# Boese0601/RC-MVSNet

Hardware: AMD Instinct MI355X
Metric: ref-scenes/sec (DTU 3-view 512x640, D=48/32/8) (higher is better)
Workload: dtype f32; 1 GPU; BASELINE configs[1]: CascadeMVSNet_eval.forward, DTU-shaped 3 views 512x640, D=(48,32,8), batch 1 per GPU, fp32, random-init seeded weights; views=3, height=512, width=640, parallelism=scene-per-gpu x1, ranks=1, procs_per_gpu=1, rccl_ranks=0

## Files before the change

### rc_mvsnet_amd/csrc/conv3d_deep.hip

```cpp
#include "common.h"
#include "x3_pieces.h"
#include <atomic>
#include <type_traits>

namespace rcmvs {

enum { DP_S1 = 0, DP_S2 = 1, DP_T2 = 2 };

__host__ __device__ constexpr int dp_ntaps(int p) { return (((p >> 2) & 1) + 1) * (((p >> 1) & 1) + 1) * ((p & 1) + 1); }
__host__ __device__ constexpr int dp_first_sum(int p) { int s = 0; for (int q = 0; q < p; ++q) s += dp_ntaps(q); return s; }
__host__ __device__ constexpr int dp_first(int p) { return (int)((0x130F0B0905030100ull >> (8 * p)) & 0xffu); }
static_assert(dp_first(1) == dp_first_sum(1) && dp_first(2) == dp_first_sum(2) && dp_first(3) == dp_first_sum(3) && dp_first(4) == dp_first_sum(4) &&
              dp_first(5) == dp_first_sum(5) && dp_first(6) == dp_first_sum(6) && dp_first(7) == dp_first_sum(7) && dp_first(0) == 0, "class offsets");
__host__ __device__ inline void dp_class_tap(int p, int i, int& kd, int& kh, int& kw) {
    const int pd = (p >> 2) & 1, ph = (p >> 1) & 1, pw = p & 1;
    const int iw = i & pw, ih = (i >> pw) & ph, id = (i >> (pw + ph)) & pd;
    kd = pd ? 2 * id : 1; kh = ph ? 2 * ih : 1; kw = pw ? 2 * iw : 1;
}

template <int CIN, int COUT, int KIND, int MS = 1>
struct Deep {
    static constexpr int NT = 2;
    static constexpr int TH = 2 * NT, TW = 8;
    static constexpr int MT = COUT / 16;
    static constexpr int HALVES = CIN >= 32 ? CIN / 32 : 1;
    static constexpr int TPS = CIN >= 32 ? 1 : 32 / CIN;
    static constexpr int HD = KIND == DP_T2 ? 2 : 3;
    static constexpr int HH = KIND == DP_S1 ? TH + 2 : (KIND == DP_S2 ? 2 * TH + 1 : TH + 1);
    static constexpr int HW = KIND == DP_S1 ? TW + 2 : (KIND == DP_S2 ? 2 * TW + 1 : TW + 1);
    static constexpr int CS = KIND == DP_S2 ? 2 : 1;
    static constexpr int NVOX = HD * HH * HW;
    static constexpr int VS = CIN * 2 + 16;
    static constexpr int PLANE = NVOX * VS;
    static constexpr int KSTEPS = (27 + TPS - 1) / TPS * HALVES;
    static constexpr int UNITS = NVOX * (CIN / 8);
    static constexpr int NLD = (UNITS + 511) / 512;
    static constexpr int PF = KIND == DP_T2 ? 6 : 8;
    static constexpr int MSPLIT = (KIND != DP_T2 && MT == 4) ? MS : 1;
    static constexpr int MB = MT / MSPLIT;
    static constexpr int KP = KIND == DP_T2 ? 1 : 8 / MB;
    static constexpr int PARTB = KIND == DP_T2 ? 0 : (KP - 1) * MB * NT * 1024;
    static constexpr int LDS = 2 * PLANE + PARTB + 64;
    static constexpr long long IMG_HALFS = 8 + (long long)KSTEPS * 2 * MT * 512;
    static_assert((CIN % 32 == 0 || (CIN == 16 && KIND != DP_T2)) && COUT % 16 == 0 && (KIND == DP_T2 ? (MT == 2 || MT == 1) : (MT == 4 || MT == 2)), "wave layout");
};

template <int CIN, int COUT, int KIND>
__global__ void deep_pack_kernel(const float* __restrict__ w, unsigned short* __restrict__ img, int transposed, const float* __restrict__ wsc) {
    using C = Deep<CIN, COUT, KIND>;
    const int t = blockIdx.x * blockDim.x + threadIdx.x;
    if (t >= C::KSTEPS * C::MT * 512) return;
    const int e = t & 7, lane = (t >> 3) & 63, mt = (t >> 9) % C::MT, j = (t >> 9) / C::MT;
    const int co = mt * 16 + (lane & 15), kq = lane >> 4;
    int tap, half;
    if (KIND == DP_T2) {
        int p = 0;
        while (p < 7 && j >= dp_first(p + 1) * C::HALVES) ++p;
        const int jj = j - dp_first(p) * C::HALVES;
        int kd, kh, kw;
        dp_class_tap(p, jj / C::HALVES, kd, kh, kw);
        tap = (kd * 3 + kh) * 3 + kw;
        half = jj % C::HALVES;
    } else if (C::TPS == 2) { tap = 2 * j + (kq >> 1); half = 0; }
    else { tap = j / C::HALVES; half = j % C::HALVES; }
    const int ci = C::TPS == 2 ? (kq & 1) * 8 + e : half * 32 + kq * 8 + e;
    float v = 0.0f;
    if (tap < 27) v = transposed ? w[((long long)ci * COUT + co) * 27 + (transposed == 2 ? 26 - tap : tap)] : w[((long long)co * CIN + ci) * 27 + tap];
    const float sw = wsc[0];
    if (t == 0) { float* hdr = reinterpret_cast<float*>(img); hdr[0] = sw; hdr[1] = wsc[1]; hdr[2] = 0.0f; hdr[3] = 0.0f; }
    const float vs = v * sw;
    const _Float16 h = (_Float16)vs;
    const _Float16 l = (_Float16)(vs - (float)h);
    const long long base = 8 + (((long long)j * 2) * C::MT + mt) * 512 + lane * 8 + e;
    img[base] = __builtin_bit_cast(unsigned short, h);
    img[base + (long long)C::MT * 512] = __builtin_bit_cast(unsigned short, l);
}

struct DeepDims {
    int B, D, H, W;
    int Dg, Hg, Wg;
    int Do, Ho, Wo;
    int tiles_h, tiles_w, relu;
};

__device__ __forceinline__ int dp_t2_segments(int wave, int (&cls)[3]) {
    const int g = wave >> 1;
    cls[0] = g == 0 ? 7 : (g == 1 ? 3 : (g == 2 ? 5 : 6));
    cls[1] = g == 1 ? 1 : (g == 2 ? 2 : 4);
    cls[2] = 0;
    return g == 0 ? 1 : (g == 1 ? 3 : 2);
}

template <int CIN, int COUT, int KIND, int MS = 1>
__global__ __launch_bounds__(512) void conv3d_deep_kernel(
    const float* __restrict__ x, const x3_u32x4* __restrict__ wimg, const float* __restrict__ scale, const float* __restrict__ shift,
    const float* __restrict__ res, float* __restrict__ y, DeepDims dm, const float* __restrict__ xmax, float* __restrict__ ymax) {
    using C = Deep<CIN, COUT, KIND, MS>;
    constexpr int MT = C::MT, NT = C::NT, PF = C::PF, VS = C::VS, PLANE = C::PLANE, HALVES = C::HALVES;
    constexpr int OOB = 0x7ffffff0;
    extern __shared__ __attribute__((aligned(16))) x3_byte smem[];
    x3_byte* const part = smem + 2 * PLANE;
    float* const redmax = reinterpret_cast<float*>(part + C::PARTB);
    const int tid = threadIdx.x, lane = tid & 63;
    const int wave = __builtin_amdgcn_readfirstlane(tid >> 6);
    const int n = lane & 15, kq = lane >> 4;
    int bt = blockIdx.x;
    const int tw = bt % dm.tiles_w; bt /= dm.tiles_w;
    const int th = bt % dm.tiles_h; bt /= dm.tiles_h;
    const int dg = bt % dm.Dg, b = bt / dm.Dg;
    const int h0 = th * C::TH, w0 = tw * C::TW;
    const int zd0 = KIND == DP_S1 ? dg - 1 : (KIND == DP_S2 ? 2 * dg - 1 : dg);
    const int zh0 = KIND == DP_S1 ? h0 - 1 : (KIND == DP_S2 ? 2 * h0 - 1 : h0);
    const int zw0 = KIND == DP_S1 ? w0 - 1 : (KIND == DP_S2 ? 2 * w0 - 1 : w0);
    const float xmax_lane = xmax[lane * 16];
    const float whdr = reinterpret_cast<const float*>(wimg)[1];

    int seg_cls[3] = {0, 0, 0}, nseg = 1, mt0;
    if constexpr (KIND == DP_T2 && MT == 1) { seg_cls[0] = wave; mt0 = 0; }
    else if constexpr (KIND == DP_T2) { nseg = dp_t2_segments(wave, seg_cls); mt0 = wave & 1; }
    else mt0 = blockIdx.y * C::MB + wave % C::MB;
    const int kp = KIND == DP_T2 ? 0 : wave / C::MB;
    const int mtl = KIND == DP_T2 ? 0 : wave % C::MB;
    auto seg_range = [&](int sg, int& j0, int& nsteps) {
        if constexpr (KIND == DP_T2) {
            const int cls = seg_cls[sg], nt = dp_ntaps(cls);
            const bool drop = (cls & 4) && zd0 + 1 >= dm.D;
            j0 = (dp_first(cls) + (drop ? nt / 2 : 0)) * HALVES;
            nsteps = (drop ? nt / 2 : nt) * HALVES;
        } else {
            const int lo = (zd0 < 0 ? 9 : 0) * HALVES / C::TPS, hi = ((zd0 + 2 >= dm.D ? 18 : 27) * HALVES + C::TPS - 1) / C::TPS, per = (hi - lo + C::KP - 1) / C::KP;
            j0 = min(lo + kp * per, hi);
            nsteps = min(per, hi - j0);
        }
    };
    auto tap_offset = [&](int cls, int j) -> int {
        const int half = j % HALVES;
        int od, oh, ow;
        if constexpr (KIND == DP_T2) {
            int kd, kh, kw;
            dp_class_tap(cls, j / HALVES - dp_first(cls), kd, kh, kw);
            od = kd == 0; oh = kh == 0; ow = kw == 0;
        } else { const int tp = j / HALVES; od = tp / 9; oh = (tp / 3) % 3; ow = tp % 3; }
        return ((od * C::HH + oh) * C::HW + ow) * VS + half * 64;
    };
    auto tap_offset_of = [&](int tp) -> int { tp = min(tp, 26); return (((tp / 9) * C::HH + (tp / 3) % 3) * C::HW + tp % 3) * VS; };

    __amdgpu_buffer_rsrc_t wrs = __builtin_amdgcn_make_buffer_rsrc(const_cast<x3_u32x4*>(wimg + 1), (short)0, (int)(C::KSTEPS * 2 * MT * 1024), 0x00020000);
    constexpr int NR = KIND == DP_T2 ? 2 : 1;
    x3_u32x4 ah[NR][PF], al[NR][PF];
    const int alane = lane * 16 + mt0 * 1024;
    auto load_a = [&](auto ring, int slot, int j0, int nsteps, int jj) {
        constexpr int R = decltype(ring)::value;
        const int so = (j0 + jj) * (2 * MT * 1024);
        const int vo = jj < nsteps ? alane : OOB;
        ah[R][slot] = __builtin_amdgcn_raw_buffer_load_b128(wrs, vo, so, 0);
        al[R][slot] = __builtin_amdgcn_raw_buffer_load_b128(wrs, vo == OOB ? OOB : vo + MT * 1024, so, 0);
    };
    using Ring0 = std::integral_constant<int, 0>;
    using Ring1 = std::integral_constant<int, NR - 1>;

    float unscale;
    {
        __amdgpu_buffer_rsrc_t xrs = __builtin_amdgcn_make_buffer_rsrc(const_cast<float*>(x), (short)0,
                                                                       (int)((long long)dm.B * dm.D * dm.H * dm.W * CIN * 4), 0x00020000);
        x3_f32x4 pf[C::NLD][2];
        int lo_[C::NLD];
#pragma unroll
        for (int i = 0; i < C::NLD; ++i) {
            const int u = tid + i * 512;
            const int vox = u / (CIN / 8), cu = u % (CIN / 8);
            const int hw_ = vox % C::HW, hh = (vox / C::HW) % C::HH, hd = vox / (C::HW * C::HH);
            const int id = zd0 + hd, ih = zh0 + hh, iw = zw0 + hw_;
            const bool in = u < C::UNITS && id >= 0 && id < dm.D && ih >= 0 && ih < dm.H && iw >= 0 && iw < dm.W;
            const int off = in ? ((((b * dm.D + id) * dm.H + ih) * dm.W + iw) * CIN + cu * 8) * 4 : OOB;
            pf[i][0] = __builtin_bit_cast(x3_f32x4, __builtin_amdgcn_raw_buffer_load_b128(xrs, off, 0, 0));
            pf[i][1] = __builtin_bit_cast(x3_f32x4, __builtin_amdgcn_raw_buffer_load_b128(xrs, in ? off + 16 : OOB, 0, 0));
            lo_[i] = u < C::UNITS ? vox * VS + cu * 16 : -1;
        }
        {
            int j0, nsteps;
            seg_range(0, j0, nsteps);
#pragma unroll
            for (int u = 0; u < PF; ++u) load_a(Ring0{}, u, j0, nsteps, u);
        }
        float bound = xmax_lane;
#pragma unroll
        for (int m = 32; m > 0; m >>= 1) bound = fmaxf(bound, __shfl_xor(bound, m));
        float xinv;
        const float xs_scale = x3_pow2_scale(bound, xinv);
        unscale = xinv * whdr;
#pragma unroll
        for (int i = 0; i < C::NLD; ++i) {
            x3_u32x2 h0_, l0_, h1_, l1_;
            x3_split4h(pf[i][0] * xs_scale, h0_, l0_);
            x3_split4h(pf[i][1] * xs_scale, h1_, l1_);
            if (lo_[i] >= 0) {
                *reinterpret_cast<x3_u32x4*>(smem + lo_[i]) = (x3_u32x4){h0_.x, h0_.y, h1_.x, h1_.y};
                *reinterpret_cast<x3_u32x4*>(smem + PLANE + lo_[i]) = (x3_u32x4){l0_.x, l0_.y, l1_.x, l1_.y};
            }
        }
    }
    __syncthreads();

    static_assert(PF % 2 == 0, "the B double buffer alternates with the step parity");
    int bb[NT];
#pragma unroll
    for (int t = 0; t < NT; ++t) bb[t] = (((2 * t + (n >> 3)) * C::CS) * C::HW + (n & 7) * C::CS) * VS + (C::TPS == 2 ? (kq & 1) : kq) * 16;
    float vmax = 0.0f;
#pragma unroll
    for (int sg = 0; sg < (KIND == DP_T2 ? 3 : 1); ++sg) {
        if (sg >= nseg) break;
        const int cls = seg_cls[sg];
        int j0, nsteps;
        seg_range(sg, j0, nsteps);
        x3_f32x4 acc[NT][3];
#pragma unroll
        for (int t = 0; t < NT; ++t)
#pragma unroll
            for (int c = 0; c < 3; ++c) acc[t][c] = (x3_f32x4){0.f, 0.f, 0.f, 0.f};
        x3_u32x4 bq[2][NT][2];
        const int jl = j0 + min(lane, nsteps - 1);
        const int entv = C::TPS == 2 ? tap_offset_of(2 * jl) : tap_offset(cls, jl);
        const int entv2 = C::TPS == 2 ? tap_offset_of(2 * jl + 1) : 0;
        auto read_b = [&](int buf, int jj) {
            int boff = __builtin_amdgcn_readlane(entv, jj);
            if constexpr (C::TPS == 2) { const int b2 = __builtin_amdgcn_readlane(entv2, jj); boff = (kq >> 1) ? b2 : boff; }
#pragma unroll
            for (int t = 0; t < NT; ++t) {
                bq[buf][t][0] = *reinterpret_cast<const x3_u32x4*>(smem + bb[t] + boff);
                bq[buf][t][1] = *reinterpret_cast<const x3_u32x4*>(smem + PLANE + bb[t] + boff);
            }
        };
        auto run = [&](auto ring, auto other) {
            constexpr int R = decltype(ring)::value;
            if (sg + 1 < nseg) {
                int j0n, nn;
                seg_range(sg + 1, j0n, nn);
#pragma unroll
                for (int u = 0; u < PF; ++u) load_a(other, u, j0n, nn, u);
            }
            auto mfmas = [&](int slot, int buf) {
#pragma unroll
                for (int t = 0; t < NT; ++t) {
                    acc[t][0] = x3_mfma<2>(ah[R][slot], bq[buf][t][0], acc[t][0]);
                    acc[t][1] = x3_mfma<2>(ah[R][slot], bq[buf][t][1], acc[t][1]);
                    acc[t][2] = x3_mfma<2>(al[R][slot], bq[buf][t][0], acc[t][2]);
                }
            };
            read_b(0, 0);
            int base = 0;
            for (; base + PF <= nsteps; base += PF) {
#pragma unroll
                for (int u = 0; u < PF; ++u) {
                    read_b((u + 1) & 1, base + u + 1);
                    __builtin_amdgcn_sched_barrier(0);
                    mfmas(u, u & 1);
                    __builtin_amdgcn_sched_barrier(0);
                    load_a(ring, u, j0, nsteps, base + u + PF);
                }
            }
#pragma unroll
            for (int u = 0; u < PF; ++u)
                if (base + u < nsteps) {
                    read_b((u + 1) & 1, base + u + 1);
                    __builtin_amdgcn_sched_barrier(0);
                    mfmas(u, u & 1);
                    __builtin_amdgcn_sched_barrier(0);
                }
        };
        if (NR == 1 || !(sg & 1)) run(Ring0{}, Ring1{});
        else run(Ring1{}, Ring0{});

        x3_f32x4 tot[NT];
#pragma unroll
        for (int t = 0; t < NT; ++t) tot[t] = acc[t][0] + (acc[t][1] + acc[t][2]);
        bool finisher = true;
        if constexpr (KIND != DP_T2) {
            finisher = kp == 0;
            if (!finisher) {
#pragma unroll
                for (int t = 0; t < NT; ++t) *reinterpret_cast<x3_f32x4*>(part + ((((kp - 1) * C::MB + mtl) * NT + t) * 64 + lane) * 16) = tot[t];
            }
            __syncthreads();
            if (finisher) {
#pragma unroll
                for (int q = 0; q < C::KP - 1; ++q)
#pragma unroll
                    for (int t = 0; t < NT; ++t) tot[t] += *reinterpret_cast<const x3_f32x4*>(part + (((q * C::MB + mtl) * NT + t) * 64 + lane) * 16);
            }
        }
        if (finisher) {
            const int pd = (cls >> 2) & 1, ph = (cls >> 1) & 1, pw = cls & 1;
            const int co = mt0 * 16 + kq * 4;
            x3_f32x4 sc = (x3_f32x4){unscale, unscale, unscale, unscale}, sh = (x3_f32x4){0.f, 0.f, 0.f, 0.f};
            if (scale) {
                sc = *reinterpret_cast<const x3_f32x4*>(scale + co) * unscale;
                sh = *reinterpret_cast<const x3_f32x4*>(shift + co);
            }
#pragma unroll
            for (int t = 0; t < NT; ++t) {
                const int ch = h0 + 2 * t + (n >> 3), cw = w0 + (n & 7);
                if (ch >= dm.Hg || cw >= dm.Wg) continue;
                const int od = KIND == DP_T2 ? 2 * dg + pd : dg, oh = KIND == DP_T2 ? 2 * ch + ph : ch, ow = KIND == DP_T2 ? 2 * cw + pw : cw;
                const long long ov = ((((long long)b * dm.Do + od) * dm.Ho + oh) * dm.Wo + ow) * COUT + co;
                x3_f32x4 v = tot[t] * sc + sh;
                if (dm.relu) v = __builtin_elementwise_max(v, (x3_f32x4){0.f, 0.f, 0.f, 0.f});
                if (res) v += *reinterpret_cast<const x3_f32x4*>(res + ov);
                *reinterpret_cast<x3_f32x4*>(y + ov) = v;
                vmax = x3_absmax4(vmax, v);
            }
        }
    }
    if (ymax) {
#pragma unroll
        for (int m = 32; m > 0; m >>= 1) vmax = fmaxf(vmax, __shfl_xor(vmax, m));
        if (lane == 0) redmax[wave] = vmax;
        __syncthreads();
        if (tid == 0) {
            float m = redmax[0];
#pragma unroll
            for (int i = 1; i < 8; ++i) m = fmaxf(m, redmax[i]);
            atomicMax(reinterpret_cast<unsigned int*>(ymax) + (blockIdx.x & 63) * 16, __float_as_uint(m));
        }
    }
}

#define RCMVS_DEEP_LIST(X) X(32, 64, DP_S2) X(64, 64, DP_S1) X(64, 32, DP_T2) X(32, 32, DP_S1) X(32, 16, DP_T2) X(16, 32, DP_S2)

bool conv3d_deep_supported(int Ci, int Co, int kind) {
    if (Ci == 16 && Co == 32) {
        static const bool on = [] { const char* e = getenv("RCMVS_DEEP3"); return !e || e[0] != '0'; }();
        if (!on) return false;
    }
    if (Ci == 32 && Co == 16) {
        static const bool on = [] { const char* e = getenv("RCMVS_DEEP9"); return !e || e[0] != '0'; }();
        if (!on) return false;
    }
    if (Ci == 32 && Co == 32) {
        static const bool on = [] { const char* e = getenv("RCMVS_DEEP4"); return !e || e[0] != '0'; }();
        if (!on) return false;
    }
#define DP_CASE(CI, CO, K) if (Ci == CI && Co == CO && kind == K) return true;
    RCMVS_DEEP_LIST(DP_CASE)
#undef DP_CASE
    return false;
}

long long conv3d_deep_weight_floats(int Ci, int Co, int kind) {
#define DP_CASE(CI, CO, K) if (Ci == CI && Co == CO && kind == K) return Deep<CI, CO, K>::IMG_HALFS / 2;
    RCMVS_DEEP_LIST(DP_CASE)
#undef DP_CASE
    return 0;
}

int conv3d_deep_pack(const float* w, float* img, int Co, int Ci, int kind, int transposed, const float* wsc, hipStream_t st) {
#define DP_CASE(CI, CO, K) if (Ci == CI && Co == CO && kind == K) { \
        const int nthr = Deep<CI, CO, K>::KSTEPS * Deep<CI, CO, K>::MT * 512; \
        hipLaunchKernelGGL((deep_pack_kernel<CI, CO, K>), dim3((nthr + 255) / 256), dim3(256), 0, st, w, reinterpret_cast<unsigned short*>(img), transposed, wsc); \
        return launch_status("conv3d_deep_pack"); }
    RCMVS_DEEP_LIST(DP_CASE)
#undef DP_CASE
    return fail(-1, "conv3d_deep_pack: unsupported Ci=%d Co=%d kind=%d", Ci, Co, kind);
}

template <int CI, int CO, int K, int MS>
static int deep_launch_ms(const float* x, const float* wimg, const float* scale, const float* shift, const float* res, float* y,
                          const DeepDims& dm, long long blocks, int dev, const float* xmax, float* ymax, hipStream_t st) {
    using C = Deep<CI, CO, K, MS>;
    constexpr int MAXDEV = 64;
    static std::atomic<bool> raised[MAXDEV];
    if (C::LDS > 64 * 1024 && !raised[dev].load(std::memory_order_acquire)) {
        if (hipFuncSetAttribute((const void*)conv3d_deep_kernel<CI, CO, K, MS>, hipFuncAttributeMaxDynamicSharedMemorySize, C::LDS) != hipSuccess)
            return fail(-1, "conv3d_deep: cannot raise the dynamic LDS limit to %d bytes", C::LDS);
        raised[dev].store(true, std::memory_order_release);
    }
    hipLaunchKernelGGL((conv3d_deep_kernel<CI, CO, K, MS>), dim3((unsigned)blocks, C::MSPLIT), dim3(512), C::LDS, st, x, reinterpret_cast<const x3_u32x4*>(wimg),
                       scale, shift, res, y, dm, xmax, ymax);
    return launch_status("conv3d_deep");
}

template <int CI, int CO, int K>
static int deep_launch_t(const float* x, const float* wimg, const float* scale, const float* shift, const float* res, float* y,
                         const DeepDims& dm_in, int dev, const float* xmax, float* ymax, hipStream_t st) {
    using C = Deep<CI, CO, K>;
    DeepDims dm = dm_in;
    dm.tiles_h = (dm.Hg + C::TH - 1) / C::TH; dm.tiles_w = (dm.Wg + C::TW - 1) / C::TW;
    const long long blocks = (long long)dm.B * dm.Dg * dm.tiles_h * dm.tiles_w;
    if (blocks <= 0 || blocks > 0x7fffffffLL) return fail(-1, "conv3d_deep: bad grid");
    if constexpr (K != DP_T2 && CO == 64) {
        static std::atomic<int> cu_of[64];
        if (cu_of[dev] == 0) {
            hipDeviceProp_t prop;
            cu_of[dev] = (hipGetDeviceProperties(&prop, dev) == hipSuccess && prop.multiProcessorCount > 0) ? prop.multiProcessorCount : 256;
        }
        if (2 * blocks <= cu_of[dev].load()) return deep_launch_ms<CI, CO, K, 2>(x, wimg, scale, shift, res, y, dm, blocks, dev, xmax, ymax, st);
    }
    return deep_launch_ms<CI, CO, K, 1>(x, wimg, scale, shift, res, y, dm, blocks, dev, xmax, ymax, st);
}

int conv3d_deep_launch(const float* x, const float* wimg, const float* scale, const float* shift, const float* res, float* y,
                       int B, int D, int H, int W, int Ci, int Co, int kind, int relu, hipStream_t st, const float* xmax, float* ymax) {
    if (!xmax) return fail(-1, "conv3d_deep: the fp16-pair form needs a bound of max|x|");
    DeepDims dm;
    dm.B = B; dm.D = D; dm.H = H; dm.W = W; dm.relu = relu;
    if (kind == DP_T2) { dm.Do = 2 * D; dm.Ho = 2 * H; dm.Wo = 2 * W; dm.Dg = D; dm.Hg = H; dm.Wg = W; }
    else {
        const int s = kind == DP_S2 ? 2 : 1;
        dm.Do = (D - 1) / s + 1; dm.Ho = (H - 1) / s + 1; dm.Wo = (W - 1) / s + 1;
        dm.Dg = dm.Do; dm.Hg = dm.Ho; dm.Wg = dm.Wo;
    }
    if ((long long)B * D * H * W * Ci * 4 >= 0x7ffffff0LL) return fail(-1, "conv3d_deep: input tensor too large for 32-bit offsets");
    dm.tiles_h = dm.tiles_w = 0;
    int dev = 0;
    if (hipGetDevice(&dev) != hipSuccess || dev < 0 || dev >= 64) return fail(-1, "conv3d_deep: cannot query the device");
#define DP_CASE(CI, CO, K) if (Ci == CI && Co == CO && kind == K) return deep_launch_t<CI, CO, K>(x, wimg, scale, shift, res, y, dm, dev, xmax, ymax, st);
    RCMVS_DEEP_LIST(DP_CASE)
#undef DP_CASE
    return fail(-1, "conv3d_deep: unsupported Ci=%d Co=%d kind=%d", Ci, Co, kind);
}

}
```

Before: 982.1 ref-scenes/s.

## Re-layout deep conv3d LDS planes with row padding to cut bank conflicts

Moves the Deep tile config into a shared header and changes the LDS activation-plane layout. It adds per-row padding and a per-CIN voxel stride, de-interleaves even and odd columns for the stride-2 CIN=32 case, and remaps the global-load unit order so LDS writes group better. The goal is to reduce LDS bank conflicts in the B-operand reads and the staging writes of the MFMA conv. It also adds a host-side bank-conflict model header, used only for analysis. The cost is extra LDS footprint from padding, which may lower occupancy, plus more complex index arithmetic in the load loop.

```diff
diff --git a/rc_mvsnet_amd/csrc/conv3d_deep.hip b/rc_mvsnet_amd/csrc/conv3d_deep.hip
--- a/rc_mvsnet_amd/csrc/conv3d_deep.hip
+++ b/rc_mvsnet_amd/csrc/conv3d_deep.hip
@@ -1,49 +1,10 @@
 #include "common.h"
 #include "x3_pieces.h"
+#include "deep_lds.h"
 #include <atomic>
 #include <type_traits>
 
 namespace rcmvs {
-
-enum { DP_S1 = 0, DP_S2 = 1, DP_T2 = 2 };
-
-__host__ __device__ constexpr int dp_ntaps(int p) { return (((p >> 2) & 1) + 1) * (((p >> 1) & 1) + 1) * ((p & 1) + 1); }
-__host__ __device__ constexpr int dp_first_sum(int p) { int s = 0; for (int q = 0; q < p; ++q) s += dp_ntaps(q); return s; }
-__host__ __device__ constexpr int dp_first(int p) { return (int)((0x130F0B0905030100ull >> (8 * p)) & 0xffu); }
-static_assert(dp_first(1) == dp_first_sum(1) && dp_first(2) == dp_first_sum(2) && dp_first(3) == dp_first_sum(3) && dp_first(4) == dp_first_sum(4) &&
-              dp_first(5) == dp_first_sum(5) && dp_first(6) == dp_first_sum(6) && dp_first(7) == dp_first_sum(7) && dp_first(0) == 0, "class offsets");
-__host__ __device__ inline void dp_class_tap(int p, int i, int& kd, int& kh, int& kw) {
-    const int pd = (p >> 2) & 1, ph = (p >> 1) & 1, pw = p & 1;
-    const int iw = i & pw, ih = (i >> pw) & ph, id = (i >> (pw + ph)) & pd;
-    kd = pd ? 2 * id : 1; kh = ph ? 2 * ih : 1; kw = pw ? 2 * iw : 1;
-}
-
-template <int CIN, int COUT, int KIND, int MS = 1>
-struct Deep {
-    static constexpr int NT = 2;
-    static constexpr int TH = 2 * NT, TW = 8;
-    static constexpr int MT = COUT / 16;
-    static constexpr int HALVES = CIN >= 32 ? CIN / 32 : 1;
-    static constexpr int TPS = CIN >= 32 ? 1 : 32 / CIN;
-    static constexpr int HD = KIND == DP_T2 ? 2 : 3;
-    static constexpr int HH = KIND == DP_S1 ? TH + 2 : (KIND == DP_S2 ? 2 * TH + 1 : TH + 1);
-    static constexpr int HW = KIND == DP_S1 ? TW + 2 : (KIND == DP_S2 ? 2 * TW + 1 : TW + 1);
-    static constexpr int CS = KIND == DP_S2 ? 2 : 1;
-    static constexpr int NVOX = HD * HH * HW;
-    static constexpr int VS = CIN * 2 + 16;
-    static constexpr int PLANE = NVOX * VS;
-    static constexpr int KSTEPS = (27 + TPS - 1) / TPS * HALVES;
-    static constexpr int UNITS = NVOX * (CIN / 8);
-    static constexpr int NLD = (UNITS + 511) / 512;
-    static constexpr int PF = KIND == DP_T2 ? 6 : 8;
-    static constexpr int MSPLIT = (KIND != DP_T2 && MT == 4) ? MS : 1;
-    static constexpr int MB = MT / MSPLIT;
-    static constexpr int KP = KIND == DP_T2 ? 1 : 8 / MB;
-    static constexpr int PARTB = KIND == DP_T2 ? 0 : (KP - 1) * MB * NT * 1024;
-    static constexpr int LDS = 2 * PLANE + PARTB + 64;
-    static constexpr long long IMG_HALFS = 8 + (long long)KSTEPS * 2 * MT * 512;
-    static_assert((CIN % 32 == 0 || (CIN == 16 && KIND != DP_T2)) && COUT % 16 == 0 && (KIND == DP_T2 ? (MT == 2 || MT == 1) : (MT == 4 || MT == 2)), "wave layout");
-};
 
 template <int CIN, int COUT, int KIND>
 __global__ void deep_pack_kernel(const float* __restrict__ w, unsigned short* __restrict__ img, int transposed, const float* __restrict__ wsc) {
@@ -96,7 +57,7 @@
     const float* __restrict__ x, const x3_u32x4* __restrict__ wimg, const float* __restrict__ scale, const float* __restrict__ shift,
     const float* __restrict__ res, float* __restrict__ y, DeepDims dm, const float* __restrict__ xmax, float* __restrict__ ymax) {
     using C = Deep<CIN, COUT, KIND, MS>;
-    constexpr int MT = C::MT, NT = C::NT, PF = C::PF, VS = C::VS, PLANE = C::PLANE, HALVES = C::HALVES;
+    constexpr int MT = C::MT, NT = C::NT, PF = C::PF, PLANE = C::PLANE, HALVES = C::HALVES;
     constexpr int OOB = 0x7ffffff0;
     extern __shared__ __attribute__((aligned(16))) x3_byte smem[];
     x3_byte* const part = smem + 2 * PLANE;
@@ -141,9 +102,9 @@
             dp_class_tap(cls, j / HALVES - dp_first(cls), kd, kh, kw);
             od = kd == 0; oh = kh == 0; ow = kw == 0;
         } else { const int tp = j / HALVES; od = tp / 9; oh = (tp / 3) % 3; ow = tp % 3; }
-        return ((od * C::HH + oh) * C::HW + ow) * VS + half * 64;
+        return C::tap_off(od, oh, ow, half);
     };
-    auto tap_offset_of = [&](int tp) -> int { tp = min(tp, 26); return (((tp / 9) * C::HH + (tp / 3) % 3) * C::HW + tp % 3) * VS; };
+    auto tap_offset_of = [&](int tp) -> int { tp = min(tp, 26); return C::tap_off(tp / 9, (tp / 3) % 3, tp % 3, 0); };
 
     __amdgpu_buffer_rsrc_t wrs = __builtin_amdgcn_make_buffer_rsrc(const_cast<x3_u32x4*>(wimg + 1), (short)0, (int)(C::KSTEPS * 2 * MT * 1024), 0x00020000);
     constexpr int NR = KIND == DP_T2 ? 2 : 1;
@@ -167,15 +128,15 @@
         int lo_[C::NLD];
 #pragma unroll
         for (int i = 0; i < C::NLD; ++i) {
-            const int u = tid + i * 512;
-            const int vox = u / (CIN / 8), cu = u % (CIN / 8);
-            const int hw_ = vox % C::HW, hh = (vox / C::HW) % C::HH, hd = vox / (C::HW * C::HH);
+            int hr, hw_, cu;
+            const bool live = C::unit(tid + i * 512, hr, hw_, cu);
+            const int hh = hr % C::HH, hd = hr / C::HH;
             const int id = zd0 + hd, ih = zh0 + hh, iw = zw0 + hw_;
-            const bool in = u < C::UNITS && id >= 0 && id < dm.D && ih >= 0 && ih < dm.H && iw >= 0 && iw < dm.W;
+            const bool in = live && id >= 0 && id < dm.D && ih >= 0 && ih < dm.H && iw >= 0 && iw < dm.W;
             const int off = in ? ((((b * dm.D + id) * dm.H + ih) * dm.W + iw) * CIN + cu * 8) * 4 : OOB;
             pf[i][0] = __builtin_bit_cast(x3_f32x4, __builtin_amdgcn_raw_buffer_load_b128(xrs, off, 0, 0));
             pf[i][1] = __builtin_bit_cast(x3_f32x4, __builtin_amdgcn_raw_buffer_load_b128(xrs, in ? off + 16 : OOB, 0, 0));
-            lo_[i] = u < C::UNITS ? vox * VS + cu * 16 : -1;
+            lo_[i] = live ? C::vox_off(hr, hw_, cu) : -1;
         }
         {
             int j0, nsteps;
@@ -205,7 +166,7 @@
     static_assert(PF % 2 == 0, "the B double buffer alternates with the step parity");
     int bb[NT];
 #pragma unroll
-    for (int t = 0; t < NT; ++t) bb[t] = (((2 * t + (n >> 3)) * C::CS) * C::HW + (n & 7) * C::CS) * VS + (C::TPS == 2 ? (kq & 1) : kq) * 16;
+    for (int t = 0; t < NT; ++t) bb[t] = C::cell_off(t, n, C::TPS == 2 ? (kq & 1) : kq);
     float vmax = 0.0f;
 #pragma unroll
     for (int sg = 0; sg < (KIND == DP_T2 ? 3 : 1); ++sg) {
@@ -279,14 +240,14 @@
             finisher = kp == 0;
             if (!finisher) {
 #pragma unroll
-                for (int t = 0; t < NT; ++t) *reinterpret_cast<x3_f32x4*>(part + ((((kp - 1) * C::MB + mtl) * NT + t) * 64 + lane) * 16) = tot[t];
+                for (int t = 0; t < NT; ++t) *reinterpret_cast<x3_f32x4*>(part + C::part_off(kp - 1, mtl, t, lane)) = tot[t];
             }
             __syncthreads();
             if (finisher) {
 #pragma unroll
                 for (int q = 0; q < C::KP - 1; ++q)
 #pragma unroll
-                    for (int t = 0; t < NT; ++t) tot[t] += *reinterpret_cast<const x3_f32x4*>(part + (((q * C::MB + mtl) * NT + t) * 64 + lane) * 16);
+                    for (int t = 0; t < NT; ++t) tot[t] += *reinterpret_cast<const x3_f32x4*>(part + C::part_off(q, mtl, t, lane));
             }
         }
         if (finisher) {
diff --git a/rc_mvsnet_amd/csrc/deep_lds.h b/rc_mvsnet_amd/csrc/deep_lds.h
--- /dev/null
+++ b/rc_mvsnet_amd/csrc/deep_lds.h
@@ -0,0 +1,78 @@
+#pragma once
+
+#ifndef __HIPCC__
+#ifndef __host__
+#define __host__
+#endif
+#ifndef __device__
+#define __device__
+#endif
+#endif
+
+namespace rcmvs {
+
+enum { DP_S1 = 0, DP_S2 = 1, DP_T2 = 2 };
+
+__host__ __device__ constexpr int dp_ntaps(int p) { return (((p >> 2) & 1) + 1) * (((p >> 1) & 1) + 1) * ((p & 1) + 1); }
+__host__ __device__ constexpr int dp_first_sum(int p) { int s = 0; for (int q = 0; q < p; ++q) s += dp_ntaps(q); return s; }
+__host__ __device__ constexpr int dp_first(int p) { return (int)((0x130F0B0905030100ull >> (8 * p)) & 0xffu); }
+static_assert(dp_first(1) == dp_first_sum(1) && dp_first(2) == dp_first_sum(2) && dp_first(3) == dp_first_sum(3) && dp_first(4) == dp_first_sum(4) &&
+              dp_first(5) == dp_first_sum(5) && dp_first(6) == dp_first_sum(6) && dp_first(7) == dp_first_sum(7) && dp_first(0) == 0, "class offsets");
+__host__ __device__ inline void dp_class_tap(int p, int i, int& kd, int& kh, int& kw) {
+    const int pd = (p >> 2) & 1, ph = (p >> 1) & 1, pw = p & 1;
+    const int iw = i & pw, ih = (i >> pw) & ph, id = (i >> (pw + ph)) & pd;
+    kd = pd ? 2 * id : 1; kh = ph ? 2 * ih : 1; kw = pw ? 2 * iw : 1;
+}
+
+template <int CIN, int COUT, int KIND, int MS = 1>
+struct Deep {
+    static constexpr int NT = 2;
+    static constexpr int TH = 2 * NT, TW = 8;
+    static constexpr int MT = COUT / 16;
+    static constexpr int HALVES = CIN >= 32 ? CIN / 32 : 1;
+    static constexpr int TPS = CIN >= 32 ? 1 : 32 / CIN;
+    static constexpr int HD = KIND == DP_T2 ? 2 : 3;
+    static constexpr int HH = KIND == DP_S1 ? TH + 2 : (KIND == DP_S2 ? 2 * TH + 1 : TH + 1);
+    static constexpr int HW = KIND == DP_S1 ? TW + 2 : (KIND == DP_S2 ? 2 * TW + 1 : TW + 1);
+    static constexpr int CS = KIND == DP_S2 ? 2 : 1;
+    static constexpr int ROWS = HD * HH;
+    static constexpr int NVOX = ROWS * HW;
+
+    static constexpr int VS = CIN == 64 ? 160 : 2 * CIN;
+    static constexpr int RPAD = CIN == 64 ? (KIND == DP_T2 ? 96 : 192) : (KIND == DP_S2 ? 16 : 32);
+    static constexpr bool XDEINT = CIN == 32 && KIND == DP_S2;
+    static constexpr int XODD = (HW + 1) / 2;
+    static constexpr int RS = HW * VS + RPAD;
+    static constexpr int PLANE = ROWS * RS;
+    static constexpr int CPV = CIN / 8;
+    static constexpr int GQ = CIN == 64 ? 8 : (CIN == 32 ? 4 : 2);
+    static constexpr int GV = 8 / GQ;
+    static constexpr int HWU = (CIN == 64 || (CIN == 32 && KIND == DP_S1)) ? HW : HW + 1;
+    static constexpr int UNITS = (ROWS * HWU + GV - 1) / GV * GV * CPV;
+    static constexpr int NLD = (UNITS + 511) / 512;
+
+    static constexpr int KSTEPS = (27 + TPS - 1) / TPS * HALVES;
+    static constexpr int PF = KIND == DP_T2 ? 6 : 8;
+    static constexpr int MSPLIT = (KIND != DP_T2 && MT == 4) ? MS : 1;
+    static constexpr int MB = MT / MSPLIT;
+    static constexpr int KP = KIND == DP_T2 ? 1 : 8 / MB;
+    static constexpr int PARTB = KIND == DP_T2 ? 0 : (KP - 1) * MB * NT * 1024;
+    static constexpr int LDS = 2 * PLANE + PARTB + 64;
+    static constexpr long long IMG_HALFS = 8 + (long long)KSTEPS * 2 * MT * 512;
+    static_assert((CIN % 32 == 0 || (CIN == 16 && KIND != DP_T2)) && COUT % 16 == 0 && (KIND == DP_T2 ? (MT == 2 || MT == 1) : (MT == 4 || MT == 2)), "wave layout");
+    static_assert(VS >= 2 * CIN && VS % 16 == 0 && RS % 16 == 0 && GQ <= CPV && HWU >= HW, "piece plane layout");
+
+    __host__ __device__ static constexpr int vox_off(int r, int x, int q) { return r * RS + (XDEINT ? (x & 1) * XODD + (x >> 1) : x) * VS + q * 16; }
+    __host__ __device__ static constexpr bool unit(int u, int& r, int& x, int& q) {
+        const int blk = u / (GV * CPV), rem = u % (GV * CPV);
+        const int v = blk * GV + (rem % 8) / GQ;
+        const int pos = v % HWU;
+        r = v / HWU; x = XDEINT ? (pos < XODD ? 2 * pos : 2 * (pos - XODD) + 1) : pos; q = (rem / 8) * GQ + rem % GQ;
+        return r < ROWS && pos < HW;
+    }
+    __host__ __device__ static constexpr int cell_off(int t, int n, int q) { return vox_off((2 * t + (n >> 3)) * CS, (n & 7) * CS, q); }
+    __host__ __device__ static constexpr int tap_off(int od, int oh, int ow, int half) { return vox_off(od * HH + oh, ow, half * 4); }
+    __host__ __device__ static constexpr int part_off(int part, int mtl, int t, int lane) { return (((part * MB + mtl) * NT + t) * 64 + lane) * 16; }
+};
+
+}
diff --git a/rc_mvsnet_amd/csrc/lds_banks.h b/rc_mvsnet_amd/csrc/lds_banks.h
--- /dev/null
+++ b/rc_mvsnet_amd/csrc/lds_banks.h
@@ -0,0 +1,44 @@
+#pragma once
+#include <algorithm>
+#include <vector>
+
+namespace rcmvs {
+namespace lds_banks {
+
+enum Op { READ_B32, READ_B64, READ_B128, WRITE_B32, WRITE_B64, WRITE_B128 };
+
+inline int op_bytes(Op op) { return (op == READ_B32 || op == WRITE_B32) ? 4 : ((op == READ_B64 || op == WRITE_B64) ? 8 : 16); }
+inline int op_banks(Op op) { return (op == READ_B64 || op == READ_B128) ? 64 : 32; }
+
+inline int groups(Op op) { return op == READ_B128 || op == WRITE_B64 ? 4 : (op == WRITE_B128 ? 8 : 2); }
+inline int group_of(Op op, int lane) {
+    if (op == READ_B128) {
+        const int l = lane & 31;
+        const bool first = l < 4 || (l >= 12 && l < 16) || (l >= 20 && l < 28);
+        return (lane >> 5) * 2 + (first ? 0 : 1);
+    }
+    if (op == WRITE_B64) return lane >> 4;
+    if (op == WRITE_B128) return lane >> 3;
+    return lane >> 5;
+}
+
+inline int ways(Op op, const int (&off)[64]) {
+    const int nb = op_banks(op), dwords = op_bytes(op) / 4;
+    int worst = 1;
+    for (int g = 0; g < groups(op); ++g) {
+        std::vector<std::vector<int>> on(nb);
+        for (int lane = 0; lane < 64; ++lane) {
+            if (off[lane] < 0 || group_of(op, lane) != g) continue;
+            for (int d = 0; d < dwords; ++d) {
+                const int dw = off[lane] / 4 + d;
+                std::vector<int>& v = on[dw % nb];
+                if (std::find(v.begin(), v.end(), dw) == v.end()) v.push_back(dw);
+            }
+        }
+        for (const std::vector<int>& v : on) worst = std::max(worst, (int)v.size());
+    }
+    return worst;
+}
+
+}
+}
```

Result: no change. 987.3 ref-scenes/s, median of 6 (+0.5%).
